# pmh47/dirt

Hardware: AMD Instinct MI355X
Metric: forward+backward Mpixels/s at 1024x1024x4ch, 10k-tri mesh (higher is better)
Workload: dtype f32 (f64 edge functions); 1 GPU; K3: rand_mesh F=10000 at 1024x1024x4, 1 scene(s) per GPU, forward+backward; scenes_per_gpu=1, parallelism=batch-sharded x1, no collective, launch=eager (Python wrapper + C ABI per step)

## Files before the change

dirt_amd/csrc/dirt_device.h:

```cpp
#pragma once
#include <hip/hip_runtime.h>
#include <stdint.h>

namespace dirt {

template <class T>
__device__ __forceinline__ T ld_off(const void* base, uint32_t off)
{
    return *reinterpret_cast<const T*>(reinterpret_cast<const char*>(base) + off);
}
template <class T>
__device__ __forceinline__ void st_off(void* base, uint32_t off, T v)
{
    *reinterpret_cast<T*>(reinterpret_cast<char*>(base) + off) = v;
}

typedef uint32_t dirt_u32x4 __attribute__((ext_vector_type(4)));
template <class T>
__device__ __forceinline__ void st_off_wt(void* base, uint32_t off, T v)
{
    static_assert(sizeof(T) == 16 || sizeof(T) == 8, "write-through stores: 16 or 8 bytes");
    if constexpr (sizeof(T) == 16) {
        dirt_u32x4 d;
        __builtin_memcpy(&d, &v, 16);
        __builtin_amdgcn_raw_buffer_store_b128(d, __builtin_amdgcn_make_buffer_rsrc(base, 0, -1, 0x00020000), (int)off, 0, 16);
    } else {
        unsigned long long d;
        __builtin_memcpy(&d, &v, 8);
        __hip_atomic_store(reinterpret_cast<unsigned long long*>(reinterpret_cast<char*>(base) + off), d, __ATOMIC_RELAXED, __HIP_MEMORY_SCOPE_AGENT);
    }
}
template <bool WT, class T>
__device__ __forceinline__ void st_off_if(void* base, uint32_t off, T v)
{
    if constexpr (WT) st_off_wt<T>(base, off, v);
    else st_off<T>(base, off, v);
}

struct Float3 { float x, y, z; };

struct alignas(128) FaceRec {
    double coef[9];
    double inv_det;
    uint32_t flags;
    int32_t vid[3];
    double zp[3];
    uint32_t pad0;
    uint32_t pad1;
};
static_assert(sizeof(FaceRec) == 128, "FaceRec must be 128 bytes");
constexpr int FACE_SHADE_BYTES = 96;

constexpr uint32_t FACE_VALID = 0x80000000u;

struct alignas(8) FaceBox {
    int16_t i_min, i_max, r_min, r_max;
};
static_assert(sizeof(FaceBox) == 8, "FaceBox must be 8 bytes");

constexpr uint32_t Z24_CLEAR = 0x00FFFFFFu;

__device__ __forceinline__ void face_fetch_indices(const int32_t* __restrict__ face, int32_t (&idx)[3])
{
    idx[0] = face[0]; idx[1] = face[1]; idx[2] = face[2];
}
__device__ __forceinline__ void face_fetch_vertices(const float* __restrict__ verts, int V, const int32_t (&idx)[3], float4 (&vv)[3])
{
#pragma unroll
    for (int k = 0; k < 3; ++k)
        vv[k] = V > 0 ? *reinterpret_cast<const float4*>(verts + (size_t)((uint32_t)idx[k] < (uint32_t)V ? idx[k] : 0) * 4) : make_float4(0.f, 0.f, 0.f, 0.f);
}
__device__ inline bool setup_face_from(const float4 (&vv)[3], const int32_t (&idx)[3], int V, int H, int W, FaceRec& rec, FaceBox& box);

__device__ inline bool setup_face(const float* __restrict__ verts, int V, const int32_t* __restrict__ face,
                                  int H, int W, FaceRec& rec, FaceBox& box)
{
    int32_t idx[3];
    float4 vv[3];
    face_fetch_indices(face, idx);
    face_fetch_vertices(verts, V, idx, vv);
    return setup_face_from(vv, idx, V, H, W, rec, box);
}

__device__ inline bool setup_face_edges(const float4 (&vv)[3], const int32_t (&idx)[3], int V, int H, int W, FaceRec& rec)
{
    double X[3], Y[3], Wc[3], Z[3];
    const int32_t i0 = idx[0], i1 = idx[1], i2 = idx[2];
    const bool index_ok = ((uint32_t)i0 < (uint32_t)V) & ((uint32_t)i1 < (uint32_t)V) & ((uint32_t)i2 < (uint32_t)V);
    if (V <= 0) return false;
    if (!index_ok) return false;
#pragma unroll
    for (int k = 0; k < 3; ++k) {
        const int32_t vi = k == 0 ? i0 : (k == 1 ? i1 : i2);
        const float4 v = vv[k];
        if (!(isfinite(v.x) && isfinite(v.y) && isfinite(v.z) && isfinite(v.w))) return false;
        X[k] = ((double)v.x + (double)v.w) * (0.5 * (double)W);
        Y[k] = ((double)v.y + (double)v.w) * (0.5 * (double)H);
        Wc[k] = (double)v.w;
        Z[k] = (double)v.z;
        rec.vid[k] = vi;
    }
    double a[3], b[3], c[3];
#pragma unroll
    for (int k = 0; k < 3; ++k) {
        const int p = (k + 1) % 3, q = (k + 2) % 3;
        double m1, m2;
        m1 = Y[p] * Wc[q]; m2 = Wc[p] * Y[q]; a[k] = m1 - m2;
        m1 = Wc[p] * X[q]; m2 = X[p] * Wc[q]; b[k] = m1 - m2;
        m1 = X[p] * Y[q];  m2 = Y[p] * X[q];  c[k] = m1 - m2;
    }
    const double t0 = X[0] * a[0], t1 = Y[0] * b[0], t2 = Wc[0] * c[0];
    double det = (t0 + t1) + t2;
    if (!isfinite(det) || det == 0.0) return false;
    if (det < 0.0) {
#pragma unroll
        for (int k = 0; k < 3; ++k) { a[k] = -a[k]; b[k] = -b[k]; c[k] = -c[k]; }
        det = -det;
    }
    const double inv_det = 1.0 / det;
    if (!isfinite(inv_det)) return false;

    double zs[3];
#pragma unroll
    for (int k = 0; k < 3; ++k) zs[k] = Z[k] * inv_det;
    {
        double m0, m1, m2;
        m0 = a[0] * zs[0]; m1 = a[1] * zs[1]; m2 = a[2] * zs[2]; rec.zp[0] = ((m0 + m1) + m2) * 8388607.5;
        m0 = b[0] * zs[0]; m1 = b[1] * zs[1]; m2 = b[2] * zs[2]; rec.zp[1] = ((m0 + m1) + m2) * 8388607.5;
        m0 = c[0] * zs[0]; m1 = c[1] * zs[1]; m2 = c[2] * zs[2]; rec.zp[2] = fma((m0 + m1) + m2, 8388607.5, 8388607.5);
    }
    uint32_t flags = FACE_VALID;
#pragma unroll
    for (int k = 0; k < 3; ++k) {
        const bool incl = (a[k] > 0.0) || (a[k] == 0.0 && b[k] > 0.0);
        if (!incl) { a[k] = -a[k]; b[k] = -b[k]; c[k] = -c[k]; flags |= (1u << k); }
        rec.coef[3 * k + 0] = a[k]; rec.coef[3 * k + 1] = b[k]; rec.coef[3 * k + 2] = c[k];
    }
    rec.flags = flags; rec.pad0 = 0; rec.pad1 = 0;
    rec.inv_det = inv_det;
    return true;
}

__device__ inline bool setup_face_box(const float4 (&vv)[3], int H, int W, FaceBox& box)
{
    double X[3], Y[3], Wc[3], Z[3];
#pragma unroll
    for (int k = 0; k < 3; ++k) {
        const float4 v = vv[k];
        X[k] = ((double)v.x + (double)v.w) * (0.5 * (double)W);
        Y[k] = ((double)v.y + (double)v.w) * (0.5 * (double)H);
        Wc[k] = (double)v.w;
        Z[k] = (double)v.z;
    }
    const int npos = (Wc[0] > 0.0) + (Wc[1] > 0.0) + (Wc[2] > 0.0);
    if (npos == 0) return false;
    int i_min = 0, i_max = W - 1, j_min = 0, j_max = H - 1;
    if (npos == 3) {
        if (Z[0] > Wc[0] && Z[1] > Wc[1] && Z[2] > Wc[2]) return false;
        if (Z[0] < -Wc[0] && Z[1] < -Wc[1] && Z[2] < -Wc[2]) return false;
        float xmin = INFINITY, xmax = -INFINITY, ymin = INFINITY, ymax = -INFINITY;
#pragma unroll
        for (int k = 0; k < 3; ++k) {
            const float rw = 1.0f / (float)Wc[k];
            float xw = (float)X[k] * rw, yw = (float)Y[k] * rw;
            if (!(fabsf(xw) <= 32768.f)) xw = xw > 0.f ? 32768.f : -32768.f;
            if (!(fabsf(yw) <= 32768.f)) yw = yw > 0.f ? 32768.f : -32768.f;
            xmin = fminf(xmin, xw); xmax = fmaxf(xmax, xw);
            ymin = fminf(ymin, yw); ymax = fmaxf(ymax, yw);
        }
        if (!(xmin <= xmax) || !(ymin <= ymax)) { xmin = ymin = -32768.f; xmax = ymax = 32768.f; }
        const float d = 1.0f / 32.0f;
        float lo, hi;
        lo = ceilf(fmaxf(xmin - 0.5f - d, -1.0f)); hi = floorf(fminf(xmax - 0.5f + d, (float)W));
        if (lo > (float)i_min) i_min = (int)lo;
        if (hi < (float)i_max) i_max = (int)hi;
        lo = ceilf(fmaxf(ymin - 0.5f - d, -1.0f)); hi = floorf(fminf(ymax - 0.5f + d, (float)H));
        if (lo > (float)j_min) j_min = (int)lo;
        if (hi < (float)j_max) j_max = (int)hi;
    }
    if (i_min > i_max || j_min > j_max) return false;
    box.i_min = (int16_t)i_min; box.i_max = (int16_t)i_max;
    box.r_min = (int16_t)(H - 1 - j_max); box.r_max = (int16_t)(H - 1 - j_min);
    return true;
}

__device__ inline bool setup_face_from(const float4 (&vv)[3], const int32_t (&idx)[3], int V, int H, int W, FaceRec& rec, FaceBox& box)
{
    if (!setup_face_edges(vv, idx, V, H, W, rec)) return false;
    return setup_face_box(vv, H, W, box);
}

__device__ inline void edge_eval(const double* coef, double px, double py, double F[3])
{
    F[0] = fma(coef[0], px, fma(coef[1], py, coef[2]));
    F[1] = fma(coef[3], px, fma(coef[4], py, coef[5]));
    F[2] = fma(coef[6], px, fma(coef[7], py, coef[8]));
}

__device__ inline void bary_eval(const double F[3], uint32_t flags, double inv_det, float b[3], float& clip_w)
{
    const float l0 = __uint_as_float(__float_as_uint((float)(F[0] * inv_det)) ^ (flags << 31));
    const float l1 = __uint_as_float(__float_as_uint((float)(F[1] * inv_det)) ^ ((flags << 30) & 0x80000000u));
    const float l2 = __uint_as_float(__float_as_uint((float)(F[2] * inv_det)) ^ ((flags << 29) & 0x80000000u));
    const float s = (l0 + l1) + l2;
    const float r = 1.0f / s;
    b[0] = l0 * r; b[1] = l1 * r; b[2] = l2 * r;
    clip_w = r;
}

__device__ __forceinline__ float2 encode_bary(float b0, float b1, float b2)
{
    const bool omit2 = (b2 >= b0) & (b2 >= b1);
    const bool omit0 = !omit2 & (b0 >= b1);
    const bool omit1 = !omit2 & !omit0;
    const float p = omit2 ? b0 : (omit0 ? b1 : b2);
    const float q = omit2 ? b1 : (omit0 ? b2 : b0);
    return make_float2(__uint_as_float(__float_as_uint(p) | (omit0 ? 0x80000000u : 0u)),
                       __uint_as_float(__float_as_uint(q) | (omit1 ? 0x80000000u : 0u)));
}
__device__ __forceinline__ void decode_bary(float2 e, float (&b)[3])
{
    const bool sp = (int32_t)__float_as_uint(e.x) < 0, sq = (int32_t)__float_as_uint(e.y) < 0;
    const float P = fabsf(e.x), Q = fabsf(e.y);
    const float d = (1.f - P) - Q;
    b[0] = sq ? Q : (sp ? d : P);
    b[1] = sq ? d : (sp ? P : Q);
    b[2] = sq ? P : (sp ? Q : d);
}

__device__ __forceinline__ int xcd_tile(int b, int ntiles)
{
    const int x = b & 7, j = b >> 3;
    const int q = ntiles >> 3, rem = ntiles & 7;
    return x * q + min(x, rem) + j;
}

inline uint32_t tile_magic(int tiles_x) { return tiles_x <= 1 ? 0u : (uint32_t)(0x100000000ull / (uint32_t)tiles_x) + 1u; }
template <class Params>
inline void set_tile_grid(Params& p, int tile_w, int tile_h)
{
    p.tiles_x = (p.W + tile_w - 1) / tile_w;
    p.tiles_y = (p.H + tile_h - 1) / tile_h;
    p.tiles_x_magic = tile_magic(p.tiles_x);
}
__device__ __forceinline__ void tile_xy(int tile, int tiles_x, uint32_t magic, int& tx, int& ty)
{
    ty = magic ? (int)__umulhi((uint32_t)tile, magic) : tile;
    tx = tile - ty * tiles_x;
}

}
```

dirt_amd/csrc/dirt_forward.hip:

```cpp
#include <type_traits>
#include "dirt_device.h"
#include "dirt_launch.h"
#include "dirt_raster_common.h"
#include "../../include/dirt_hip.h"

namespace dirt {

#ifdef DIRT_TRACE
__device__ long long* g_trace_fwd_setup = nullptr;
__device__ long long* g_trace_fwd_raster = nullptr;
extern "C" void dirt_debug_set_trace_forward(void* ps, void* pr)
{
    long long* q = reinterpret_cast<long long*>(ps);
    (void)hipMemcpyToSymbol(HIP_SYMBOL(g_trace_fwd_setup), &q, sizeof(q));
    q = reinterpret_cast<long long*>(pr);
    (void)hipMemcpyToSymbol(HIP_SYMBOL(g_trace_fwd_raster), &q, sizeof(q));
}
#define FMARK() do { if (tr_n < 12) { long long t_; asm volatile("s_memtime %0\n\ts_waitcnt lgkmcnt(0)" : "=s"(t_) :: "memory"); tr_t[tr_n++] = t_; } } while (0)
#define FTRACE_DECL() long long tr_t[12]; int tr_n = 0; const long long tr_wall0 = wall_clock64()
#else
#define FMARK() do {} while (0)
#define FTRACE_DECL() do {} while (0)
#endif

namespace {

constexpr int MAX_FACE_BINS = 16;

__device__ __forceinline__ void glds16(const void* base, uint32_t voff, uint32_t lds_addr)
{
    unsigned keep;
    asm volatile("s_mov_b32 %0, m0\n\ts_mov_b32 m0, %3\n\ts_nop 0\n\tglobal_load_lds_dwordx4 %1, %2\n\ts_mov_b32 m0, %0"
                 : "=&s"(keep) : "v"(voff), "s"(base), "s"(lds_addr) : "memory");
}

#define DIRT_LDS __attribute__((address_space(3)))

constexpr int WAIT_VMCNT_0 = 0x0F70;

template <class T>
__device__ __forceinline__ uint32_t lds_address(T* p)
{
    return (uint32_t)(uintptr_t)(__attribute__((address_space(3))) void*)p;
}

typedef float f32x4 __attribute__((ext_vector_type(4)));
typedef double f64x2 __attribute__((ext_vector_type(2)));
typedef uint32_t u32x4 __attribute__((ext_vector_type(4)));
static_assert(offsetof(TileRec, bound) == 36 && offsetof(TileRec, box) == 40 && offsetof(TileRec, zp) == 48 && offsetof(TileRec, face) == 72,
              "fetch_rec reads TileRec by offsets");

__device__ __forceinline__ TileRec fetch_rec(const TileRec* rec)
{
    const volatile DIRT_LDS char* q = (const volatile DIRT_LDS char*)rec;
    const f32x4 p0 = *(const volatile DIRT_LDS f32x4*)(q + 0);
    const f32x4 p1 = *(const volatile DIRT_LDS f32x4*)(q + 16);
    const u32x4 p2 = *(const volatile DIRT_LDS u32x4*)(q + 32);
    const f64x2 p3 = *(const volatile DIRT_LDS f64x2*)(q + 48);
    const u32x4 p4 = *(const volatile DIRT_LDS u32x4*)(q + 64);
    TileRec t;
    t.a[0] = p0.x; t.a[1] = p0.y; t.a[2] = p0.z; t.b[0] = p0.w;
    t.b[1] = p1.x; t.b[2] = p1.y; t.c[0] = p1.z; t.c[1] = p1.w;
    t.c[2] = __uint_as_float(p2.x); t.bound = __uint_as_float(p2.y);
    t.box.i_min = (int16_t)(p2.z & 0xFFFFu); t.box.i_max = (int16_t)(p2.z >> 16);
    t.box.r_min = (int16_t)(p2.w & 0xFFFFu); t.box.r_max = (int16_t)(p2.w >> 16);
    t.zp[0] = p3.x; t.zp[1] = p3.y; t.zp[2] = __longlong_as_double((long long)(((unsigned long long)p4.y << 32) | p4.x));
    t.face = (int32_t)p4.z; t.flags = p4.w;
    return t;
}

}

constexpr int STHREADS = 256;
template <int CK>
__global__ __launch_bounds__(STHREADS) void setup_kernel_v2(const float* __restrict__ a_vertices, const int32_t* __restrict__ a_faces,
                                                            const float* __restrict__ a_vertex_colors, int a_shared_faces, int a_V, int a_F,
                                                            GeomParams g_in)
{
    GeomParams g = g_in;
    g.vertices = a_vertices; g.faces = a_faces; g.vertex_colors = a_vertex_colors; g.shared_faces = a_shared_faces; g.V = a_V; g.F = a_F;
    __shared__ __align__(16) unsigned long long s_mask[MAX_BINS_MASKED + 2];
    __shared__ __align__(16) FaceRec s_recs[64];
    __shared__ __align__(16) TileRec s_lrecs[64];
    __shared__ __align__(16) float4 s_crecs[CK ? 3 * 64 : 1];
    __shared__ FaceBox s_box[64];
    __shared__ uint8_t s_ok_edges[64], s_ok_box[64];
    const int ib = blockIdx.y, chunk = blockIdx.x, tid = threadIdx.x, lane = tid & 63;
    const int role = __builtin_amdgcn_readfirstlane(tid >> 6);
    FTRACE_DECL();
    FMARK();
    const int nbins = g.grid.bins_x * g.grid.bins_y, big = g.grid.big;
    BinCell* __restrict__ row = g.cells + ((size_t)ib * g.nchunk + chunk) * (size_t)g.grid.cell_chunk_stride;
    if (g.F == 0 || g.V <= 0) {
        for (int i = tid; i <= big; i += STHREADS) if (i < nbins || i == big) row[i] = BinCell{0u, 0u};
        return;
    }
    const int f0 = chunk * 64;
    const int nf = min(64, g.F - f0);
    const size_t n0 = (size_t)ib * g.F + f0;
    const int f = f0 + lane;
    const bool have = lane < nf;
    const int fs = have ? f : 0;
    const float* __restrict__ verts = g.vertices + (size_t)ib * g.V * 4;
    const float* __restrict__ cols = CK ? g.vertex_colors + (size_t)ib * g.V * CK : nullptr;
    auto fetch = [&](int vid) {
        if (role != 3) return *reinterpret_cast<const float4*>(verts + (size_t)vid * 4);
        if constexpr (CK == 0) return make_float4(0.f, 0.f, 0.f, 0.f);
        else {
            const float* __restrict__ cp = cols + (size_t)vid * CK;
            if constexpr (CK == 4) return *reinterpret_cast<const float4*>(cp);
            else if constexpr (CK == 3) { const Float3 q = *reinterpret_cast<const Float3*>(cp); return make_float4(q.x, q.y, q.z, 0.f); }
            else return make_float4(cp[0], 0.f, 0.f, 0.f);
        }
    };
    int32_t idx[3] = {0, 0, 0};
    float4 vv[3];
    const bool fetches = role != 2 && (role != 3 || CK != 0);
    if (fetches) {
        const int32_t* __restrict__ fp = g.faces + (g.shared_faces ? (size_t)fs : (size_t)ib * g.F + fs) * 3;
        idx[0] = fp[0]; idx[1] = fp[1]; idx[2] = fp[2];
#pragma unroll
        for (int k = 0; k < 3; ++k) vv[k] = fetch(min(3 * fs + k, g.V - 1));
    } else if (role == 2) {
        for (int i = lane; i < nbins; i += 64) s_mask[i] = 0ull;
        if (lane == 0) s_mask[big] = 0ull;
    }
    FMARK();
    if (fetches) {
        const bool identity = 3 * fs + 2 < g.V && idx[0] == 3 * fs && idx[1] == 3 * fs + 1 && idx[2] == 3 * fs + 2;
        if (__builtin_amdgcn_ballot_w64(have && !identity) != 0ull) {
#pragma unroll
            for (int k = 0; k < 3; ++k) {
                const int ci = identity ? 3 * fs + k : ((uint32_t)idx[k] < (uint32_t)g.V ? idx[k] : 0);
                vv[k] = fetch(ci);
            }
        }
    }
    FMARK();
    bool ok_mine = false;
    FaceBox box;
    box.i_min = 0; box.i_max = -1; box.r_min = 0; box.r_max = -1;
    if (role == 0) {
        FaceRec rec;
        ok_mine = have && setup_face_edges(vv, idx, g.V, g.H, g.W, rec);
        if (ok_mine) s_recs[lane] = rec;
        else s_recs[lane].flags = 0;
        s_ok_edges[lane] = ok_mine ? 1 : 0;
    } else if (role == 1) {
        ok_mine = have && setup_face_box(vv, g.H, g.W, box);
        s_box[lane] = box;
        s_ok_box[lane] = ok_mine ? 1 : 0;
    } else if (role == 3) {
        if constexpr (CK != 0) { s_crecs[3 * lane] = vv[0]; s_crecs[3 * lane + 1] = vv[1]; s_crecs[3 * lane + 2] = vv[2]; }
    }
    FMARK();
    __syncthreads();
    if (role == 1) {
        if (ok_mine && s_ok_edges[lane]) {
            const unsigned long long bit = 1ull << lane;
            const int bx0 = box.i_min >> g.grid.shift, bx1 = box.i_max >> g.grid.shift;
            const int by0 = box.r_min >> g.grid.shift, by1 = box.r_max >> g.grid.shift;
            if ((bx1 - bx0 + 1) * (by1 - by0 + 1) <= MAX_FACE_BINS) {
                for (int by = by0; by <= by1; ++by)
                    for (int bx = bx0; bx <= bx1; ++bx) atomicOr(&s_mask[by * g.grid.bins_x + bx], bit);
            } else {
                atomicOr(&s_mask[big], bit);
            }
            if (!g.v2_only) {
                BinEntry e;
                e.box = box; e.face = f; e.pad = 0;
                g.entries[((size_t)ib * g.nchunk + chunk) * (5 * (size_t)g.chunk_faces) + lane] = e;
            }
        }
    } else if (role == 2) {
        if (have && s_ok_edges[lane] && s_ok_box[lane]) {
            TileRec lr;
            make_local_rec(s_recs[lane], f, s_box[lane], g.H, (float)g.W, (float)g.H, &lr);
            s_lrecs[lane] = lr;
        }
    } else if (role == 0) {
        const uint4* __restrict__ src = reinterpret_cast<const uint4*>(&s_recs[0]);
        uint4* __restrict__ dst = reinterpret_cast<uint4*>(g.recs + n0);
        for (int i = lane; i < 8 * nf; i += 64) dst[i] = src[i];
    } else {
        if constexpr (CK != 0) {
            const uint4* __restrict__ src = reinterpret_cast<const uint4*>(&s_crecs[0]);
            uint4* __restrict__ dst = reinterpret_cast<uint4*>(g.crecs + 3 * n0);
            for (int i = lane; i < 3 * nf; i += 64) dst[i] = src[i];
        }
    }
    __syncthreads();
    FMARK();
    {
        const uint4* __restrict__ src = reinterpret_cast<const uint4*>(&s_lrecs[0]);
        uint4* __restrict__ dst = reinterpret_cast<uint4*>(g.lrecs + n0);
        for (int i = tid; i < 5 * nf; i += STHREADS) dst[i] = src[i];
    }
    for (int i = 2 * tid; i < nbins; i += 2 * STHREADS) {
        if (i + 1 < nbins) {
            const ulonglong2 m = *reinterpret_cast<const ulonglong2*>(&s_mask[i]);
            *reinterpret_cast<ulonglong2*>(&row[i]) = m;
        } else {
            const unsigned long long m = s_mask[i];
            row[i] = BinCell{(uint32_t)m, (uint32_t)(m >> 32)};
        }
    }
    if (tid == STHREADS - 1) {
        const unsigned long long m = s_mask[big];
        row[big] = BinCell{(uint32_t)m, (uint32_t)(m >> 32)};
    }
    FMARK();
#ifdef DIRT_TRACE
    if (tid == 0 && g_trace_fwd_setup) {
        long long* o = g_trace_fwd_setup + ((size_t)blockIdx.y * gridDim.x + blockIdx.x) * 16;
        for (int i = 0; i < 12; ++i) o[i] = i < tr_n ? tr_t[i] : 0;
        o[12] = tr_wall0; o[13] = (long long)wall_clock64() - tr_wall0;
    }
#endif
}

hipError_t launch_geometry_v2(const GeomParams& g, hipStream_t stream)
{
    const dim3 grid((unsigned)g.nchunk, (unsigned)g.B);
    const int ck = g.crecs ? g.C : 0;
    if (ck == 4) hipLaunchKernelGGL(setup_kernel_v2<4>, grid, dim3(STHREADS), 0, stream, g.vertices, g.faces, g.vertex_colors, g.shared_faces, g.V, g.F, g);
    else if (ck == 3) hipLaunchKernelGGL(setup_kernel_v2<3>, grid, dim3(STHREADS), 0, stream, g.vertices, g.faces, g.vertex_colors, g.shared_faces, g.V, g.F, g);
    else if (ck == 1) hipLaunchKernelGGL(setup_kernel_v2<1>, grid, dim3(STHREADS), 0, stream, g.vertices, g.faces, g.vertex_colors, g.shared_faces, g.V, g.F, g);
    else hipLaunchKernelGGL(setup_kernel_v2<0>, grid, dim3(STHREADS), 0, stream, g.vertices, g.faces, g.vertex_colors, g.shared_faces, g.V, g.F, g);
    return hipGetLastError();
}

namespace {

#ifndef DIRT_V2_CAP
#define DIRT_V2_CAP 96
#endif
constexpr int V2_CAP = DIRT_V2_CAP;

template <bool COLOURS>
struct alignas(16) ShadeSlot {
    double coef[9];
    double inv_det;
    uint32_t flags;
    int32_t vid[3];
    float4 col[COLOURS ? 3 : 0];
};
static_assert(sizeof(ShadeSlot<true>) == 144 && sizeof(ShadeSlot<false>) == 96, "16-byte pieces: 6 of the record, 3 colours");

}

#ifndef DIRT_V2_WAVES
#define DIRT_V2_WAVES 6
#endif
template <int MODE, int CSPEC, int WAVES = 4>
__global__ __launch_bounds__(64 * WAVES, WAVES == 8 ? 8 : DIRT_V2_WAVES) void raster_kernel_v2(
    const BinCell* __restrict__ a_cells, int a_nchunk, int a_tiles_x, int a_tiles_y, uint32_t a_tiles_x_magic, int a_shift, int a_bins_x,
    int a_big, int a_chunk_stride, RasterParams p_in)
{
    RasterParams p = p_in;
    p.cells = a_cells; p.nchunk = a_nchunk; p.tiles_x = a_tiles_x; p.tiles_y = a_tiles_y; p.tiles_x_magic = a_tiles_x_magic;
    p.grid.shift = a_shift; p.grid.bins_x = a_bins_x; p.grid.big = a_big; p.grid.cell_chunk_stride = a_chunk_stride;
    constexpr int NB = 2, NBY = WAVES == 8 ? 1 : 2, TILE = 32, PPL = NB * NBY, THREADS = 64 * WAVES, RH = 8 * NBY;
    constexpr bool COLOURS = MODE == 0;
    constexpr bool WT = WAVES == 8 && CSPEC == 4;
    constexpr int SPARTS = COLOURS ? 9 : 6;
    using Slot = ShadeSlot<COLOURS>;
    __shared__ __align__(16) TileRec s_rec[V2_CAP];
    __shared__ __align__(16) Slot s_shade[V2_CAP];
    __shared__ int32_t s_face[V2_CAP];
    __shared__ uint32_t s_count;
    FTRACE_DECL();
    FMARK();
#ifdef DIRT_TRACE
    int tr_cand = 0;
#endif
    const int tid = threadIdx.x;
    const int lane = tid & 63;
    const int wave = __builtin_amdgcn_readfirstlane(tid >> 6);
    const int ib = blockIdx.y;
    const int tile = xcd_tile(blockIdx.x, p.tiles_x * p.tiles_y);
    int tile_col, tile_row;
    tile_xy(tile, p.tiles_x, p.tiles_x_magic, tile_col, tile_row);
    const int tx0 = tile_col * TILE, tr0 = tile_row * TILE;
    constexpr int C = CSPEC;

    const FaceRec* __restrict__ recs = p.recs + (size_t)ib * p.F;
    const TileRec* __restrict__ lrecs = p.lrecs + (size_t)ib * p.F;
    const float4* __restrict__ crecs = COLOURS ? p.crecs + (size_t)ib * p.F * 3 : nullptr;
    const int bin = (tr0 >> p.grid.shift) * p.grid.bins_x + (tx0 >> p.grid.shift);
    const BinCell* __restrict__ cells = p.cells + (size_t)ib * p.nchunk * (size_t)p.grid.cell_chunk_stride;
    unsigned long long m_bin = 0ull, m_big = 0ull;
    if (tid < p.nchunk) {
        const BinCell* __restrict__ rowc = cells + (size_t)tid * p.grid.cell_chunk_stride;
        const BinCell a = rowc[bin], b = rowc[p.grid.big];
        m_bin = ((unsigned long long)a.count << 32) | a.start;
        m_big = ((unsigned long long)b.count << 32) | b.start;
    }

    const int wx = wave & 1, wy = wave >> 1;
    const int x0 = tx0 + wx * 16 + (lane & 7);
    const int r0 = tr0 + wy * RH + (lane >> 3);
    double px[NB], py[NBY];
#pragma unroll
    for (int k = 0; k < NB; ++k) px[k] = (double)(x0 + 8 * k) + 0.5;
#pragma unroll
    for (int k = 0; k < NBY; ++k) py[k] = (double)(p.H - 1 - (r0 + 8 * k)) + 0.5;
    unsigned long long best[PPL];
    int cbest[PPL];
#pragma unroll
    for (int k = 0; k < PPL; ++k) { best[k] = (unsigned long long)Z24_CLEAR << 32; cbest[k] = V2_CAP; }
    bool lds_records = true;

    const uint32_t lds_rec = (uint32_t)__builtin_amdgcn_readfirstlane((int)lds_address(&s_rec[0]));
    const uint32_t lds_shade = (uint32_t)__builtin_amdgcn_readfirstlane((int)lds_address(&s_shade[0]));

    FMARK();
    for (int round = 0;; ++round) {
        if (tid == 0) s_count = 0;
        __syncthreads();
        FMARK();
        if (64 * wave < p.nchunk) {
            const uint32_t cnt = (uint32_t)__popcll(m_bin) + (uint32_t)__popcll(m_big);
            uint32_t incl = cnt;
            incl += (uint32_t)__builtin_amdgcn_update_dpp(0, (int)incl, 0x111 , 0xF, 0xF, false);
            incl += (uint32_t)__builtin_amdgcn_update_dpp(0, (int)incl, 0x112 , 0xF, 0xF, false);
            incl += (uint32_t)__builtin_amdgcn_update_dpp(0, (int)incl, 0x114 , 0xF, 0xF, false);
            incl += (uint32_t)__builtin_amdgcn_update_dpp(0, (int)incl, 0x118 , 0xF, 0xF, false);
            incl += (uint32_t)__builtin_amdgcn_update_dpp(0, (int)incl, 0x142 , 0xA, 0xF, false);
            incl += (uint32_t)__builtin_amdgcn_update_dpp(0, (int)incl, 0x143 , 0xC, 0xF, false);
            const uint32_t total = (uint32_t)__builtin_amdgcn_readlane((int)incl, 63);
            uint32_t base = 0;
            if (total != 0u) {
                if (lane == 0) base = atomicAdd(&s_count, total);
                base = (uint32_t)__builtin_amdgcn_readfirstlane((int)base);
            }
            uint32_t slot = base + incl - cnt;
            const int face0 = tid * 64;
            while (m_bin != 0ull && slot < (uint32_t)V2_CAP) {
                s_face[slot++] = face0 + (__ffsll((long long)m_bin) - 1);
                m_bin &= m_bin - 1ull;
            }
            while (m_big != 0ull && slot < (uint32_t)V2_CAP) {
                s_face[slot++] = face0 + (__ffsll((long long)m_big) - 1);
                m_big &= m_big - 1ull;
            }
        }
        FMARK();
        __syncthreads();
        FMARK();
        const int n = (int)min(s_count, (uint32_t)V2_CAP);
        if (round != 0) lds_records = false;

        int tid_o = tid;
        asm volatile("" : "+v"(tid_o));
#pragma unroll
        for (int k = 0; k < (5 * V2_CAP + THREADS - 1) / THREADS; ++k) {
            const int idx = tid_o + THREADS * k;
            if (idx < 5 * n) {
                const int slot = idx / 5, part = idx - 5 * slot;
                glds16(lrecs, (uint32_t)s_face[slot] * (uint32_t)sizeof(TileRec) + 16u * (uint32_t)part, lds_rec + 1024u * (uint32_t)(wave + WAVES * k));
            }
        }
        asm volatile("s_waitcnt vmcnt(0)" ::: "memory");
        FMARK();
        __syncthreads();
        FMARK();
        if (round == 0) {
#pragma unroll
            for (int k = 0; k < (SPARTS * V2_CAP + THREADS - 1) / THREADS; ++k) {
// ... 221 lines not shown
```

dirt_amd/csrc/dirt_raster_common.h:

```cpp
#pragma once
#include "dirt_device.h"
#include "dirt_launch.h"

namespace dirt {

constexpr int RTHREADS = 256;
constexpr int LIST_CAP = 1024;
constexpr int SHADE_CAP = 96;
struct alignas(8) ShadeRec {
    double coef[9];
    double inv_det;
    uint32_t flags;
    int32_t vid[3];
    double pad;
};
static_assert(sizeof(ShadeRec) == 104, "ShadeRec is 26 dwords");

struct alignas(16) TileRec {
    float a[3], b[3], c[3];
    float bound;
    FaceBox box;
    double zp[3];
    int32_t face;
    uint32_t flags;
};
static_assert(sizeof(TileRec) == 80, "TileRec is 80 bytes");

__device__ __forceinline__ void make_tile_rec(const FaceRec& rec, int face, double ox, double oy, float wf, float hf, TileRec* out)
{
    const uint32_t flags = rec.flags;
    float bound = 0.f;
#pragma unroll
    for (int k = 0; k < 3; ++k) {
        const double a = rec.coef[3 * k], b = rec.coef[3 * k + 1], c = rec.coef[3 * k + 2];
        const double cl = fma(a, ox, fma(b, oy, c));
        const float sg = (flags & (1u << k)) ? -1.f : 1.f;
        const float a32 = (float)a, b32 = (float)b, c32 = (float)cl, cg = (float)c;
        const float mg = fabsf(a32) * wf + fabsf(b32) * hf + fabsf(cg);
        const float bnd = (0x1p-22f * (32.f * fabsf(a32) + 32.f * fabsf(b32) + fabsf(c32)) + 0x1p-49f * mg) * 1.0001f;
        bound = (bnd > bound || bnd != bnd) ? bnd : bound;
        out->a[k] = sg * a32; out->b[k] = sg * b32; out->c[k] = sg * c32;
    }
    out->bound = bound; out->box.i_min = 0; out->box.i_max = 0; out->box.r_min = 0; out->box.r_max = 0;
    out->zp[0] = rec.zp[0]; out->zp[1] = rec.zp[1]; out->zp[2] = rec.zp[2];
    out->flags = flags; out->face = face;
}

__device__ __forceinline__ void make_local_rec(const FaceRec& rec, int face, const FaceBox& box, int H, float wf, float hf, TileRec* out)
{
    const uint32_t flags = rec.flags;
    const double ox = (double)box.i_min + 0.5, oy = (double)(H - 1 - box.r_min) + 0.5;
    const float D = (float)(max(box.i_max - box.i_min, box.r_max - box.r_min) + 8);
    float bound = 0.f;
#pragma unroll
    for (int k = 0; k < 3; ++k) {
        const double a = rec.coef[3 * k], b = rec.coef[3 * k + 1], c = rec.coef[3 * k + 2];
        const double cl = fma(a, ox, fma(b, oy, c));
        const float sg = (flags & (1u << k)) ? -1.f : 1.f;
        const float a32 = (float)a, b32 = (float)b, c32 = (float)cl, cg = (float)c;
        const float mg = fabsf(a32) * wf + fabsf(b32) * hf + fabsf(cg);
        const float bnd = (0x1p-22f * (D * fabsf(a32) + D * fabsf(b32) + fabsf(c32)) + 0x1p-49f * mg) * 1.0001f;
        bound = (bnd > bound || bnd != bnd) ? bnd : bound;
        out->a[k] = sg * a32; out->b[k] = sg * b32; out->c[k] = sg * c32;
    }
    out->bound = bound; out->box = box;
    out->zp[0] = rec.zp[0]; out->zp[1] = rec.zp[1]; out->zp[2] = rec.zp[2];
    out->flags = flags; out->face = face;
}

template <int NB, int NBY = NB>
__device__ __forceinline__ uint32_t cull_blocks(const TileRec& t, uint32_t m4, float dx_lo0, float dy_hi0)
{
    const float nb = -t.bound;
#pragma unroll
    for (int by = 0; by < NBY; ++by) {
        const float dy_hi = dy_hi0 - 8.f * (float)by, dy_lo = dy_hi - 7.f;
#pragma unroll
        for (int bx = 0; bx < NB; ++bx) {
            const float dx_lo = dx_lo0 + 8.f * (float)bx, dx_hi = dx_lo + 7.f;
            bool out = false;
#pragma unroll
            for (int k = 0; k < 3; ++k) {
                const float e = fmaf(t.a[k], t.a[k] > 0.f ? dx_hi : dx_lo, fmaf(t.b[k], t.b[k] > 0.f ? dy_hi : dy_lo, t.c[k]));
                out |= e < nb;
            }
            if (out) m4 &= ~(1u << (NB * by + bx));
        }
    }
    return m4;
}

static __device__ __noinline__ bool covered_exact(const FaceRec* __restrict__ rec, double px, double py)
{
    const uint32_t flags = rec->flags;
    const double F0 = fma(rec->coef[0], px, fma(rec->coef[1], py, rec->coef[2]));
    const double F1 = fma(rec->coef[3], px, fma(rec->coef[4], py, rec->coef[5]));
    const double F2 = fma(rec->coef[6], px, fma(rec->coef[7], py, rec->coef[8]));
    return ((F0 >= 0.0) != ((flags & 1u) != 0)) && ((F1 >= 0.0) != ((flags & 2u) != 0)) && ((F2 >= 0.0) != ((flags & 4u) != 0));
}

template <int NB, int NBY = NB>
__device__ __forceinline__ void raster_candidate(const TileRec& t, const FaceRec* __restrict__ recs, int ci, uint32_t m4, const float* dx,
                                                 const float* dy, const double* px, const double* py, unsigned long long* best,
                                                 int* cbest)
{
#pragma unroll
    for (int by = 0; by < NBY; ++by) {
        if (!((m4 >> (NB * by)) & ((1u << NB) - 1u))) continue;
        float trow[3];
        trow[0] = fmaf(t.b[0], dy[by], t.c[0]);
        trow[1] = fmaf(t.b[1], dy[by], t.c[1]);
        trow[2] = fmaf(t.b[2], dy[by], t.c[2]);
        const double qrow = fma(t.zp[1], py[by], t.zp[2]);
#pragma unroll
        for (int bx = 0; bx < NB; ++bx) {
            const int k = NB * by + bx;
            if (!((m4 >> k) & 1u)) continue;
            const float E0 = fmaf(t.a[0], dx[bx], trow[0]);
            const float E1 = fmaf(t.a[1], dx[bx], trow[1]);
            const float E2 = fmaf(t.a[2], dx[bx], trow[2]);
            const float m = fminf(fminf(E0, E1), E2);
            unsigned long long cov_m = __builtin_amdgcn_ballot_w64(m > t.bound);
            const unsigned long long unsure_m = __builtin_amdgcn_ballot_w64(!(m < -t.bound)) & ~cov_m;
            if (__builtin_expect(unsure_m != 0ull, 0)) {
                bool c = false;
                if (__builtin_amdgcn_inverse_ballot_w64(unsure_m)) c = covered_exact(recs + t.face, px[bx], py[by]);
                cov_m |= __builtin_amdgcn_ballot_w64(c);
            }
            if (cov_m == 0ull) continue;
            const double q = fma(t.zp[0], px[bx], qrow);
            const uint32_t z24 = (uint32_t)__double_as_longlong(q + 4503599627370496.0);
            const unsigned long long in_range_m = __builtin_amdgcn_ballot_w64((unsigned long long)__double_as_longlong(q) <= 0x416FFFFFE0000000ull);
            const unsigned long long key = ((unsigned long long)z24 << 32) | (unsigned long long)(uint32_t)t.face;
            const unsigned long long wins_m = cov_m & in_range_m & __builtin_amdgcn_ballot_w64(key < best[k]);
            const bool wins = __builtin_amdgcn_inverse_ballot_w64(wins_m);
            best[k] = wins ? key : best[k];
            cbest[k] = wins ? ci : cbest[k];
        }
    }
}

__device__ __forceinline__ void raster_candidate_pair(const TileRec& t0, const TileRec& t1, const FaceRec* __restrict__ recs, int ci0, int ci1,
                                                      float dx, float dy, double px, double py, unsigned long long& best, int& cbest)
{
    const float E00 = fmaf(t0.a[0], dx, fmaf(t0.b[0], dy, t0.c[0])), E10 = fmaf(t1.a[0], dx, fmaf(t1.b[0], dy, t1.c[0]));
    const float E01 = fmaf(t0.a[1], dx, fmaf(t0.b[1], dy, t0.c[1])), E11 = fmaf(t1.a[1], dx, fmaf(t1.b[1], dy, t1.c[1]));
    const float E02 = fmaf(t0.a[2], dx, fmaf(t0.b[2], dy, t0.c[2])), E12 = fmaf(t1.a[2], dx, fmaf(t1.b[2], dy, t1.c[2]));
    const float m0 = fminf(fminf(E00, E01), E02), m1 = fminf(fminf(E10, E11), E12);
    unsigned long long cov0 = __builtin_amdgcn_ballot_w64(m0 > t0.bound), cov1 = __builtin_amdgcn_ballot_w64(m1 > t1.bound);
    const unsigned long long uns0 = __builtin_amdgcn_ballot_w64(!(m0 < -t0.bound)) & ~cov0, uns1 = __builtin_amdgcn_ballot_w64(!(m1 < -t1.bound)) & ~cov1;
    if (__builtin_expect((uns0 | uns1) != 0ull, 0)) {
        bool c0 = false, c1 = false;
        if (__builtin_amdgcn_inverse_ballot_w64(uns0)) c0 = covered_exact(recs + t0.face, px, py);
        if (__builtin_amdgcn_inverse_ballot_w64(uns1)) c1 = covered_exact(recs + t1.face, px, py);
        cov0 |= __builtin_amdgcn_ballot_w64(c0); cov1 |= __builtin_amdgcn_ballot_w64(c1);
    }
    if ((cov0 | cov1) == 0ull) return;
    const double q0 = fma(t0.zp[0], px, fma(t0.zp[1], py, t0.zp[2])), q1 = fma(t1.zp[0], px, fma(t1.zp[1], py, t1.zp[2]));
    const uint32_t z0 = (uint32_t)__double_as_longlong(q0 + 4503599627370496.0), z1 = (uint32_t)__double_as_longlong(q1 + 4503599627370496.0);
    const unsigned long long in0 = __builtin_amdgcn_ballot_w64((unsigned long long)__double_as_longlong(q0) <= 0x416FFFFFE0000000ull);
    const unsigned long long in1 = __builtin_amdgcn_ballot_w64((unsigned long long)__double_as_longlong(q1) <= 0x416FFFFFE0000000ull);
    const unsigned long long key0 = ((unsigned long long)z0 << 32) | (unsigned long long)(uint32_t)t0.face;
    const unsigned long long key1 = ((unsigned long long)z1 << 32) | (unsigned long long)(uint32_t)t1.face;
    const bool w0 = __builtin_amdgcn_inverse_ballot_w64(cov0 & in0 & __builtin_amdgcn_ballot_w64(key0 < best));
    const unsigned long long b1 = w0 ? key0 : best;
    const int c1i = w0 ? ci0 : cbest;
    const bool w1 = __builtin_amdgcn_inverse_ballot_w64(cov1 & in1 & __builtin_amdgcn_ballot_w64(key1 < b1));
    best = w1 ? key1 : b1;
    cbest = w1 ? ci1 : c1i;
}

template <bool WT = false>
__device__ __forceinline__ void store_state(float2* plane_a, float2* plane_b, uint32_t off, bool has, float b0, float b1, float b2, float clip_w, int32_t face)
{
    st_off_if<WT, float2>(plane_a, off, make_float2(has ? clip_w : INFINITY, __int_as_float(face)));
    st_off_if<WT, float2>(plane_b, off, has ? encode_bary(b0, b1, b2) : make_float2(-1.f, -1.f));
}
__device__ __forceinline__ void store_state(const RasterParams& p, size_t pix, bool has, float b0, float b1, float b2, float clip_w, int32_t face)
{
    store_state(p.state_a + pix, p.state_b + pix, 0u, has, b0, b1, b2, clip_w, face);
}

template <int NTHREADS = RTHREADS>
__device__ __forceinline__ void zero_share(void* buf, size_t bytes, unsigned per, unsigned gwg, int tid)
{
    const size_t units = bytes / 16;
    const size_t i0 = (size_t)gwg * per;
    uint4* q = reinterpret_cast<uint4*>(buf);
    for (unsigned i = (unsigned)tid; i < per; i += NTHREADS)
        if (i0 + i < units) q[i0 + i] = make_uint4(0u, 0u, 0u, 0u);
    if (gwg == 0 && (size_t)tid < (bytes % 16) / 4) reinterpret_cast<uint32_t*>(buf)[units * 4 + tid] = 0u;
}

}
```

Baseline: 26450 Mpixels/s.

## Split face setup across six wave roles with per-edge waves

The setup kernel grows from 4 to 6 waves per block. The f64 plane/depth work, each of the three edge-equation triples, the bounding box, and colors/clearing now each run in their own wave instead of one wave doing all the edge math serially. The local TileRec rows are built by the edge waves, with the bound combined through an LDS atomicMax. Bin-mask atomics and record copy-out are spread across several waves. This shortens the per-block critical path in the f64-heavy setup, at the cost of recomputing the window transform and determinant in each edge wave, larger blocks, and extra LDS atomics.

```diff
diff --git a/dirt_amd/csrc/dirt_device.h b/dirt_amd/csrc/dirt_device.h
--- a/dirt_amd/csrc/dirt_device.h
+++ b/dirt_amd/csrc/dirt_device.h
@@ -82,7 +82,30 @@
     return setup_face_from(vv, idx, V, H, W, rec, box);
 }
 
-__device__ inline bool setup_face_edges(const float4 (&vv)[3], const int32_t (&idx)[3], int V, int H, int W, FaceRec& rec)
+#define DIRT_HD __host__ __device__ __forceinline__
+
+DIRT_HD bool vertex_finite(const float4& v) { return __builtin_isfinite(v.x) && __builtin_isfinite(v.y) && __builtin_isfinite(v.z) && __builtin_isfinite(v.w); }
+DIRT_HD void vertex_window(const float4& v, int H, int W, double& X, double& Y, double& Wc)
+{
+    X = ((double)v.x + (double)v.w) * (0.5 * (double)W);
+    Y = ((double)v.y + (double)v.w) * (0.5 * (double)H);
+    Wc = (double)v.w;
+}
+DIRT_HD void edge_triple(double Xp, double Yp, double Wp, double Xq, double Yq, double Wq, double& a, double& b, double& c)
+{
+    double m1, m2;
+    m1 = Yp * Wq; m2 = Wp * Yq; a = m1 - m2;
+    m1 = Wp * Xq; m2 = Xp * Wq; b = m1 - m2;
+    m1 = Xp * Yq; m2 = Yp * Xq; c = m1 - m2;
+}
+DIRT_HD double face_det(double X0, double Y0, double W0, double a0, double b0, double c0)
+{
+    const double t0 = X0 * a0, t1 = Y0 * b0, t2 = W0 * c0;
+    return (t0 + t1) + t2;
+}
+DIRT_HD bool edge_inclusive(double a, double b) { return (a > 0.0) || (a == 0.0 && b > 0.0); }
+
+DIRT_HD bool setup_role_plane(const float4 (&vv)[3], const int32_t (&idx)[3], int V, int H, int W, FaceRec& rec)
 {
     double X[3], Y[3], Wc[3], Z[3];
     const int32_t i0 = idx[0], i1 = idx[1], i2 = idx[2];
@@ -93,10 +116,8 @@
     for (int k = 0; k < 3; ++k) {
         const int32_t vi = k == 0 ? i0 : (k == 1 ? i1 : i2);
         const float4 v = vv[k];
-        if (!(isfinite(v.x) && isfinite(v.y) && isfinite(v.z) && isfinite(v.w))) return false;
-        X[k] = ((double)v.x + (double)v.w) * (0.5 * (double)W);
-        Y[k] = ((double)v.y + (double)v.w) * (0.5 * (double)H);
-        Wc[k] = (double)v.w;
+        if (!vertex_finite(v)) return false;
+        vertex_window(v, H, W, X[k], Y[k], Wc[k]);
         Z[k] = (double)v.z;
         rec.vid[k] = vi;
     }
@@ -104,21 +125,17 @@
 #pragma unroll
     for (int k = 0; k < 3; ++k) {
         const int p = (k + 1) % 3, q = (k + 2) % 3;
-        double m1, m2;
-        m1 = Y[p] * Wc[q]; m2 = Wc[p] * Y[q]; a[k] = m1 - m2;
-        m1 = Wc[p] * X[q]; m2 = X[p] * Wc[q]; b[k] = m1 - m2;
-        m1 = X[p] * Y[q];  m2 = Y[p] * X[q];  c[k] = m1 - m2;
-    }
-    const double t0 = X[0] * a[0], t1 = Y[0] * b[0], t2 = Wc[0] * c[0];
-    double det = (t0 + t1) + t2;
-    if (!isfinite(det) || det == 0.0) return false;
+        edge_triple(X[p], Y[p], Wc[p], X[q], Y[q], Wc[q], a[k], b[k], c[k]);
+    }
+    double det = face_det(X[0], Y[0], Wc[0], a[0], b[0], c[0]);
+    if (!__builtin_isfinite(det) || det == 0.0) return false;
     if (det < 0.0) {
 #pragma unroll
         for (int k = 0; k < 3; ++k) { a[k] = -a[k]; b[k] = -b[k]; c[k] = -c[k]; }
         det = -det;
     }
     const double inv_det = 1.0 / det;
-    if (!isfinite(inv_det)) return false;
+    if (!__builtin_isfinite(inv_det)) return false;
 
     double zs[3];
 #pragma unroll
@@ -131,17 +148,43 @@
     }
     uint32_t flags = FACE_VALID;
 #pragma unroll
-    for (int k = 0; k < 3; ++k) {
-        const bool incl = (a[k] > 0.0) || (a[k] == 0.0 && b[k] > 0.0);
-        if (!incl) { a[k] = -a[k]; b[k] = -b[k]; c[k] = -c[k]; flags |= (1u << k); }
-        rec.coef[3 * k + 0] = a[k]; rec.coef[3 * k + 1] = b[k]; rec.coef[3 * k + 2] = c[k];
-    }
+    for (int k = 0; k < 3; ++k)
+        if (!edge_inclusive(a[k], b[k])) flags |= (1u << k);
     rec.flags = flags; rec.pad0 = 0; rec.pad1 = 0;
     rec.inv_det = inv_det;
     return true;
 }
 
-__device__ inline bool setup_face_box(const float4 (&vv)[3], int H, int W, FaceBox& box)
+template <int K>
+DIRT_HD bool setup_role_edge(const float4 (&vv)[3], int H, int W, double& a, double& b, double& c)
+{
+    double X[3], Y[3], Wc[3];
+#pragma unroll
+    for (int k = 0; k < 3; ++k) vertex_window(vv[k], H, W, X[k], Y[k], Wc[k]);
+    double a0, b0, c0;
+    edge_triple(X[1], Y[1], Wc[1], X[2], Y[2], Wc[2], a0, b0, c0);
+    const double det = face_det(X[0], Y[0], Wc[0], a0, b0, c0);
+    if constexpr (K == 0) { a = a0; b = b0; c = c0; }
+    else {
+        constexpr int p = (K + 1) % 3, q = (K + 2) % 3;
+        edge_triple(X[p], Y[p], Wc[p], X[q], Y[q], Wc[q], a, b, c);
+    }
+    if (det < 0.0) { a = -a; b = -b; c = -c; }
+    const bool fold = !edge_inclusive(a, b);
+    if (fold) { a = -a; b = -b; c = -c; }
+    return fold;
+}
+
+DIRT_HD bool setup_face_edges(const float4 (&vv)[3], const int32_t (&idx)[3], int V, int H, int W, FaceRec& rec)
+{
+    if (!setup_role_plane(vv, idx, V, H, W, rec)) return false;
+    setup_role_edge<0>(vv, H, W, rec.coef[0], rec.coef[1], rec.coef[2]);
+    setup_role_edge<1>(vv, H, W, rec.coef[3], rec.coef[4], rec.coef[5]);
+    setup_role_edge<2>(vv, H, W, rec.coef[6], rec.coef[7], rec.coef[8]);
+    return true;
+}
+
+DIRT_HD bool setup_face_box(const float4 (&vv)[3], int H, int W, FaceBox& box)
 {
     double X[3], Y[3], Wc[3], Z[3];
 #pragma unroll
diff --git a/dirt_amd/csrc/dirt_forward.hip b/dirt_amd/csrc/dirt_forward.hip
--- a/dirt_amd/csrc/dirt_forward.hip
+++ b/dirt_amd/csrc/dirt_forward.hip
@@ -71,7 +71,9 @@
 
 }
 
-constexpr int STHREADS = 256;
+constexpr int SWAVES = 6;
+constexpr int STHREADS = 64 * SWAVES;
+constexpr int ROLE_P = 0, ROLE_BX = 1, ROLE_E0 = 2, ROLE_E2 = 4, ROLE_C = 5;
 template <int CK>
 __global__ __launch_bounds__(STHREADS) void setup_kernel_v2(const float* __restrict__ a_vertices, const int32_t* __restrict__ a_faces,
                                                             const float* __restrict__ a_vertex_colors, int a_shared_faces, int a_V, int a_F,
@@ -87,6 +89,7 @@
     __shared__ uint8_t s_ok_edges[64], s_ok_box[64];
     const int ib = blockIdx.y, chunk = blockIdx.x, tid = threadIdx.x, lane = tid & 63;
     const int role = __builtin_amdgcn_readfirstlane(tid >> 6);
+    const bool is_edge = role >= ROLE_E0 && role <= ROLE_E2;
     FTRACE_DECL();
     FMARK();
     const int nbins = g.grid.bins_x * g.grid.bins_y, big = g.grid.big;
@@ -104,7 +107,7 @@
     const float* __restrict__ verts = g.vertices + (size_t)ib * g.V * 4;
     const float* __restrict__ cols = CK ? g.vertex_colors + (size_t)ib * g.V * CK : nullptr;
     auto fetch = [&](int vid) {
-        if (role != 3) return *reinterpret_cast<const float4*>(verts + (size_t)vid * 4);
+        if (role != ROLE_C) return *reinterpret_cast<const float4*>(verts + (size_t)vid * 4);
         if constexpr (CK == 0) return make_float4(0.f, 0.f, 0.f, 0.f);
         else {
             const float* __restrict__ cp = cols + (size_t)vid * CK;
@@ -115,15 +118,20 @@
     };
     int32_t idx[3] = {0, 0, 0};
     float4 vv[3];
-    const bool fetches = role != 2 && (role != 3 || CK != 0);
+    const bool fetches = role != ROLE_C || CK != 0;
     if (fetches) {
         const int32_t* __restrict__ fp = g.faces + (g.shared_faces ? (size_t)fs : (size_t)ib * g.F + fs) * 3;
         idx[0] = fp[0]; idx[1] = fp[1]; idx[2] = fp[2];
 #pragma unroll
         for (int k = 0; k < 3; ++k) vv[k] = fetch(min(3 * fs + k, g.V - 1));
-    } else if (role == 2) {
-        for (int i = lane; i < nbins; i += 64) s_mask[i] = 0ull;
+    }
+    if (role == ROLE_C) {
+        for (int i = 2 * lane; i < nbins; i += 128) {
+            if (i + 1 < nbins) *reinterpret_cast<ulonglong2*>(&s_mask[i]) = make_ulonglong2(0ull, 0ull);
+            else s_mask[i] = 0ull;
+        }
         if (lane == 0) s_mask[big] = 0ull;
+        s_lrecs[lane].bound = 0.f;
     }
     FMARK();
     if (fetches) {
@@ -140,53 +148,80 @@
     bool ok_mine = false;
     FaceBox box;
     box.i_min = 0; box.i_max = -1; box.r_min = 0; box.r_max = -1;
-    if (role == 0) {
+    double ea = 0.0, eb = 0.0, ec = 0.0;
+    bool efold = false;
+    if (role == ROLE_P) {
         FaceRec rec;
-        ok_mine = have && setup_face_edges(vv, idx, g.V, g.H, g.W, rec);
-        if (ok_mine) s_recs[lane] = rec;
-        else s_recs[lane].flags = 0;
+        ok_mine = have && setup_role_plane(vv, idx, g.V, g.H, g.W, rec);
+        if (ok_mine) {
+            FaceRec& r = s_recs[lane];
+            r.inv_det = rec.inv_det; r.flags = rec.flags; r.vid[0] = rec.vid[0]; r.vid[1] = rec.vid[1]; r.vid[2] = rec.vid[2];
+            r.zp[0] = rec.zp[0]; r.zp[1] = rec.zp[1]; r.zp[2] = rec.zp[2]; r.pad0 = 0; r.pad1 = 0;
+            TileRec& lr = s_lrecs[lane];
+            lr.zp[0] = rec.zp[0]; lr.zp[1] = rec.zp[1]; lr.zp[2] = rec.zp[2]; lr.face = f; lr.flags = rec.flags;
+        } else {
+            s_recs[lane].flags = 0;
+        }
         s_ok_edges[lane] = ok_mine ? 1 : 0;
-    } else if (role == 1) {
+    } else if (is_edge) {
+        if (role == ROLE_E0) efold = setup_role_edge<0>(vv, g.H, g.W, ea, eb, ec);
+        else if (role == ROLE_E0 + 1) efold = setup_role_edge<1>(vv, g.H, g.W, ea, eb, ec);
+        else efold = setup_role_edge<2>(vv, g.H, g.W, ea, eb, ec);
+        double* cf = &s_recs[lane].coef[3 * (role - ROLE_E0)];
+        cf[0] = ea; cf[1] = eb; cf[2] = ec;
+    } else if (role == ROLE_BX) {
         ok_mine = have && setup_face_box(vv, g.H, g.W, box);
         s_box[lane] = box;
+        s_lrecs[lane].box = box;
         s_ok_box[lane] = ok_mine ? 1 : 0;
-    } else if (role == 3) {
+    } else {
         if constexpr (CK != 0) { s_crecs[3 * lane] = vv[0]; s_crecs[3 * lane + 1] = vv[1]; s_crecs[3 * lane + 2] = vv[2]; }
     }
     FMARK();
     __syncthreads();
-    if (role == 1) {
-        if (ok_mine && s_ok_edges[lane]) {
-            const unsigned long long bit = 1ull << lane;
-            const int bx0 = box.i_min >> g.grid.shift, bx1 = box.i_max >> g.grid.shift;
-            const int by0 = box.r_min >> g.grid.shift, by1 = box.r_max >> g.grid.shift;
-            if ((bx1 - bx0 + 1) * (by1 - by0 + 1) <= MAX_FACE_BINS) {
-                for (int by = by0; by <= by1; ++by)
-                    for (int bx = bx0; bx <= bx1; ++bx) atomicOr(&s_mask[by * g.grid.bins_x + bx], bit);
-            } else {
-                atomicOr(&s_mask[big], bit);
-            }
-            if (!g.v2_only) {
-                BinEntry e;
-                e.box = box; e.face = f; e.pad = 0;
-                g.entries[((size_t)ib * g.nchunk + chunk) * (5 * (size_t)g.chunk_faces) + lane] = e;
-            }
-        }
-    } else if (role == 2) {
-        if (have && s_ok_edges[lane] && s_ok_box[lane]) {
-            TileRec lr;
-            make_local_rec(s_recs[lane], f, s_box[lane], g.H, (float)g.W, (float)g.H, &lr);
-            s_lrecs[lane] = lr;
-        }
-    } else if (role == 0) {
+    if (is_edge) {
+        const int k = role - ROLE_E0;
+        double ox, oy;
+        float D;
+        local_rec_origin(s_box[lane], g.H, ox, oy, D);
+        float ra, rb, rc;
+        const float bnd = local_rec_row(ea, eb, ec, efold, ox, oy, D, (float)g.W, (float)g.H, ra, rb, rc);
+        TileRec& lr = s_lrecs[lane];
+        lr.a[k] = ra; lr.b[k] = rb; lr.c[k] = rc;
+        atomicMax(reinterpret_cast<unsigned int*>(&lr.bound), __float_as_uint(bnd));
+    }
+    if (role == ROLE_P || is_edge) {
         const uint4* __restrict__ src = reinterpret_cast<const uint4*>(&s_recs[0]);
         uint4* __restrict__ dst = reinterpret_cast<uint4*>(g.recs + n0);
-        for (int i = lane; i < 8 * nf; i += 64) dst[i] = src[i];
-    } else {
+        const int w = role == ROLE_P ? 0 : role - ROLE_E0 + 1;
+        for (int i = 64 * w + lane; i < 8 * nf; i += 256) dst[i] = src[i];
+    }
+    if (!is_edge) {
+        const FaceBox fb = s_box[lane];
+        if (s_ok_box[lane] && s_ok_edges[lane]) {
+            const unsigned long long bit = 1ull << lane;
+            const int bx0 = fb.i_min >> g.grid.shift, bx1 = fb.i_max >> g.grid.shift;
+            const int by0 = fb.r_min >> g.grid.shift, by1 = fb.r_max >> g.grid.shift;
+            if ((bx1 - bx0 + 1) * (by1 - by0 + 1) <= MAX_FACE_BINS) {
+                const int ys = role == ROLE_P ? by0 + 1 : by0;
+                const int xs = role == ROLE_C ? bx0 + 1 : bx0, xstep = role == ROLE_P ? 1 : 2;
+                for (int by = ys; by <= by1; by += 2)
+                    for (int bx = xs; bx <= bx1; bx += xstep) atomicOr(&s_mask[by * g.grid.bins_x + bx], bit);
+            } else if (role == ROLE_BX) {
+                atomicOr(&s_mask[big], bit);
+            }
+            if (role == ROLE_C && !g.v2_only) {
+                BinEntry e;
+                e.box = fb; e.face = f; e.pad = 0;
+                g.entries[((size_t)ib * g.nchunk + chunk) * (5 * (size_t)g.chunk_faces) + lane] = e;
+            }
+        }
         if constexpr (CK != 0) {
-            const uint4* __restrict__ src = reinterpret_cast<const uint4*>(&s_crecs[0]);
-            uint4* __restrict__ dst = reinterpret_cast<uint4*>(g.crecs + 3 * n0);
-            for (int i = lane; i < 3 * nf; i += 64) dst[i] = src[i];
+            if (role == ROLE_C) {
+                const uint4* __restrict__ src = reinterpret_cast<const uint4*>(&s_crecs[0]);
+                uint4* __restrict__ dst = reinterpret_cast<uint4*>(g.crecs + 3 * n0);
+                for (int i = lane; i < 3 * nf; i += 64) dst[i] = src[i];
+            }
         }
     }
     __syncthreads();
@@ -211,10 +246,10 @@
     }
     FMARK();
 #ifdef DIRT_TRACE
-    if (tid == 0 && g_trace_fwd_setup) {
-        long long* o = g_trace_fwd_setup + ((size_t)blockIdx.y * gridDim.x + blockIdx.x) * 16;
+    if (lane == 0 && g_trace_fwd_setup) {
+        long long* o = g_trace_fwd_setup + (((size_t)blockIdx.y * gridDim.x + blockIdx.x) * SWAVES + role) * 16;
         for (int i = 0; i < 12; ++i) o[i] = i < tr_n ? tr_t[i] : 0;
-        o[12] = tr_wall0; o[13] = (long long)wall_clock64() - tr_wall0;
+        o[12] = tr_wall0; o[13] = (long long)wall_clock64() - tr_wall0; o[14] = SWAVES; o[15] = role;
     }
 #endif
 }
diff --git a/dirt_amd/csrc/dirt_raster_common.h b/dirt_amd/csrc/dirt_raster_common.h
--- a/dirt_amd/csrc/dirt_raster_common.h
+++ b/dirt_amd/csrc/dirt_raster_common.h
@@ -46,22 +46,34 @@
     out->flags = flags; out->face = face;
 }
 
-__device__ __forceinline__ void make_local_rec(const FaceRec& rec, int face, const FaceBox& box, int H, float wf, float hf, TileRec* out)
+DIRT_HD void local_rec_origin(const FaceBox& box, int H, double& ox, double& oy, float& D)
+{
+    ox = (double)box.i_min + 0.5; oy = (double)(H - 1 - box.r_min) + 0.5;
+    const int bw = box.i_max - box.i_min, bh = box.r_max - box.r_min;
+    D = (float)((bw > bh ? bw : bh) + 8);
+}
+DIRT_HD float local_rec_row(double a, double b, double c, bool folded, double ox, double oy, float D, float wf, float hf, float& ra, float& rb, float& rc)
+{
+    const double cl = fma(a, ox, fma(b, oy, c));
+    const float sg = folded ? -1.f : 1.f;
+    const float a32 = (float)a, b32 = (float)b, c32 = (float)cl, cg = (float)c;
+    const float mg = fabsf(a32) * wf + fabsf(b32) * hf + fabsf(cg);
+    const float bnd = (0x1p-22f * (D * fabsf(a32) + D * fabsf(b32) + fabsf(c32)) + 0x1p-49f * mg) * 1.0001f;
+    ra = sg * a32; rb = sg * b32; rc = sg * c32;
+    return bnd;
+}
+DIRT_HD void make_local_rec(const FaceRec& rec, int face, const FaceBox& box, int H, float wf, float hf, TileRec* out)
 {
     const uint32_t flags = rec.flags;
-    const double ox = (double)box.i_min + 0.5, oy = (double)(H - 1 - box.r_min) + 0.5;
-    const float D = (float)(max(box.i_max - box.i_min, box.r_max - box.r_min) + 8);
+    double ox, oy;
+    float D;
+    local_rec_origin(box, H, ox, oy, D);
     float bound = 0.f;
 #pragma unroll
     for (int k = 0; k < 3; ++k) {
-        const double a = rec.coef[3 * k], b = rec.coef[3 * k + 1], c = rec.coef[3 * k + 2];
-        const double cl = fma(a, ox, fma(b, oy, c));
-        const float sg = (flags & (1u << k)) ? -1.f : 1.f;
-        const float a32 = (float)a, b32 = (float)b, c32 = (float)cl, cg = (float)c;
-        const float mg = fabsf(a32) * wf + fabsf(b32) * hf + fabsf(cg);
-        const float bnd = (0x1p-22f * (D * fabsf(a32) + D * fabsf(b32) + fabsf(c32)) + 0x1p-49f * mg) * 1.0001f;
+        const float bnd = local_rec_row(rec.coef[3 * k], rec.coef[3 * k + 1], rec.coef[3 * k + 2], (flags & (1u << k)) != 0, ox, oy, D, wf, hf,
+                                        out->a[k], out->b[k], out->c[k]);
         bound = (bnd > bound || bnd != bnd) ? bnd : bound;
-        out->a[k] = sg * a32; out->b[k] = sg * b32; out->c[k] = sg * c32;
     }
     out->bound = bound; out->box = box;
     out->zp[0] = rec.zp[0]; out->zp[1] = rec.zp[1]; out->zp[2] = rec.zp[2];
```

Measured after the change: 26480 Mpixels/s, median of 2. About the same (+0.1%).
